# duckietown/gym-duckietown

Hardware: NVIDIA H100
Metric: env-steps/sec (obs+reward+done) at N envs, 1/2/4/8 H100 vs CPU ref (higher is better)
Workload: dtype f64 logic / f32 raster / u8 obs

## Files before the change

gym-duckietown_b200/csrc/dts_render.cu:

```cuda
#include <algorithm>
#include <cstddef>
#include <cstdlib>
#include <type_traits>
#include <vector>

#include "dts_camera.cuh"
#include "dts_kernels.h"

namespace dts {

struct FishTab {
  const int32_t* src_xy;
  const short4* cbox;
  const short4* fbox;
  const int32_t* cell_start;
  const uint16_t* cell_bins;
  const int32_t* home_start;
  const int4* home_ent;
  int ext_x, ext_y;
};

struct PilTab {
  int W, H, ow, oh;
  int tx, ty;
// ... 357 lines not shown
    cur ^= 1;
    __syncwarp();
    if (n < 3) return;
  }
  const Vtx* P = g.poly[cur];
  if (lane + 2 < n) setup_and_emit(ec, P[0], P[lane + 1], P[lane + 2], id, tex, lat);
  __syncwarp();
}

__device__ __forceinline__ void process_triangle_uniform(const EmitCtx& ec, const Vtx& a, const Vtx& b, const Vtx& c,
                                                         int id, int tex, int lat, int lane) {
  const int cls = classify(a, b, c);
  if (cls == 2) return;
  if (cls == 0) { if (lane == 0) setup_and_emit(ec, a, b, c, id, tex, lat); }
  else clip_and_emit_warp(ec, a, b, c, id, tex, lat, lane);
}

__device__ __forceinline__ void process_triangle_lanes(const EmitCtx& ec, bool have, const Vtx& a, const Vtx& b,
                                                       const Vtx& c, int id, int tex, int lat, int lane) {
  const int cls = have ? classify(a, b, c) : 2;
  if (cls == 0) setup_and_emit(ec, a, b, c, id, tex, lat);
  unsigned need = __ballot_sync(0xffffffffu, cls == 1);
  while (need) {
    const int src = __ffs(need) - 1;
    need &= need - 1;
    Vtx va, vb, vc;
    const float* fa = reinterpret_cast<const float*>(&a);
    const float* fb = reinterpret_cast<const float*>(&b);
    const float* fc = reinterpret_cast<const float*>(&c);
#pragma unroll
    for (int k = 0; k < 9; k++) {
      reinterpret_cast<float*>(&va)[k] = __shfl_sync(0xffffffffu, fa[k], src);
      reinterpret_cast<float*>(&vb)[k] = __shfl_sync(0xffffffffu, fb[k], src);
      reinterpret_cast<float*>(&vc)[k] = __shfl_sync(0xffffffffu, fc[k], src);
    }
    const int sid = __shfl_sync(0xffffffffu, id, src), stex = __shfl_sync(0xffffffffu, tex, src);
    clip_and_emit_warp(ec, va, vb, vc, sid, stex, lat, lane);
  }
}

__device__ __forceinline__ bool box_overlaps(const int qx[4], const int qy[4], int n, int x_lo, int x_hi, int y_lo, int y_hi) {
#pragma unroll
  for (int k = 0; k < 4; k++) {
    if (k >= n) break;
    const int k1 = (k + 1) & 3;
    const int dx = qx[k1] - qx[k], dy = qy[k1] - qy[k];
    const int xs = (-dy > 0) ? x_hi : x_lo;
    const int ys = (dx > 0) ? y_hi : y_lo;
    const long long e = (long long)dx * (ys - qy[k]) - (long long)dy * (xs - qx[k]);
    if (e < 0) return false;
  }
  return true;
}
__device__ __forceinline__ bool bin_overlaps(const int qx[4], const int qy[4], int n, int ox, int oy) {
  return box_overlaps(qx, qy, n, ox + 8, ox + (kCoarseW - 1) * kSub + 56, oy + 8, oy + (kCoarseH - 1) * kSub + 56);
}

constexpr unsigned kRecGround = 0x100u;
constexpr unsigned kRecFlatOk = 0x200u;
__device__ __forceinline__ unsigned build_binrec(const PrimRec* __restrict__ pr, int p, int ox, int oy, BinRec* __restrict__ out,
                                                 const short4* __restrict__ fb = nullptr) {
  const int4 w0 = __ldg(reinterpret_cast<const int4*>(pr));
  const int4 w1 = __ldg(reinterpret_cast<const int4*>(pr) + 1);
  const float4 w2 = __ldg(reinterpret_cast<const float4*>(pr) + 2);
  const int ltq = __ldg(&pr->ltq);
  const int quad = (ltq >> 24) & 1;
  const int flat = (ltq & 0xffff) ? kKindFlat : 0;
  const int qx[4] = {w0.x, w0.z, w1.x, w1.z}, qy[4] = {w0.y, w0.w, w1.y, w1.w};
  const int nv = quad ? 4 : 3;
  unsigned live = 0xffu, inside = 0xffu;
  int E0[4] = {0, 0, 0, 0}, A[4] = {0, 0, 0, 0}, B[4] = {0, 0, 0, 0};
#pragma unroll
  for (int k = 0; k < 4; k++) {
    if (k >= nv) break;
    const int ka = k, kb = (k + 1) & 3;
    const int dx = qx[kb] - qx[ka], dy = qy[kb] - qy[ka];
    const int bias = (dy > 0 || (dy == 0 && dx < 0)) ? 0 : 1;
    long long e0 = (long long)dx * (oy - qy[ka]) - (long long)dy * (ox - qx[ka]) - bias;
    if (e0 < -(1LL << 30)) live = 0;
    if (e0 > (1LL << 30)) e0 = (1LL << 30);
    if (e0 < -(1LL << 30)) e0 = -(1LL << 30);
    const int a = -dy, b = dx, e = (int)e0;
    E0[k] = e; A[k] = a; B[k] = b;
    if (fb) {
    } else {
      const int hi = (a > 0 ? a * 504 : a * 8) + (b > 0 ? b * 248 : b * 8);
      const int lo = (a > 0 ? a * 8 : a * 504) + (b > 0 ? b * 8 : b * 248);
#pragma unroll
      for (int f = 0; f < 8; f++) {
        const int ef = e + a * ((f & 3) * kBinW * kSub) + b * ((f >> 2) * kBinH * kSub);
        if (ef + hi < 0) live &= ~(1u << f);
        if (ef + lo < 0) inside &= ~(1u << f);
      }
    }
  }
  if (fb) {
#pragma unroll 1
    for (int f = 0; f < 8; f++) {
      const short4 q = fb[f];
      if (q.z < q.x) { live &= ~(1u << f); continue; }
      const int X0 = q.x * kSub - ox + 8, X1 = q.z * kSub - ox + 56, Y0 = q.y * kSub - oy + 8, Y1 = q.w * kSub - oy + 56;
#pragma unroll
      for (int k = 0; k < 4; k++) {
        if (k >= nv) break;
        const int a = A[k], b = B[k], e = E0[k];
        const int hi = (a > 0 ? a * X1 : a * X0) + (b > 0 ? b * Y1 : b * Y0);
        const int lo = (a > 0 ? a * X0 : a * X1) + (b > 0 ? b * Y0 : b * Y1);
        if (e + hi < 0) live &= ~(1u << f);
        if (e + lo < 0) inside &= ~(1u << f);
      }
    }
  }
  int tiny = 0;
  if (!fb && !quad && live) {
    const int minx = min(qx[0], min(qx[1], qx[2])) - ox, maxx = max(qx[0], max(qx[1], qx[2])) - ox;
    const int miny = min(qy[0], min(qy[1], qy[2])) - oy, maxy = max(qy[0], max(qy[1], qy[2])) - oy;
    const int x0 = max(minx >> 6, 0), x1 = min(maxx >> 6, kCoarseW - 1), y0 = max(miny >> 6, 0), y1 = min(maxy >> 6, kCoarseH - 1);
    if (x1 - x0 < 4 && y1 - y0 < 4 && x1 >= x0 && y1 >= y0) {
      tiny = kKindTiny;
      E0[3] = x0 | (y0 << 16); A[3] = x1 | (y1 << 16);
    }
  }
  const int id = __float_as_int(w2.w);
  int4* o = reinterpret_cast<int4*>(out);
  o[0] = make_int4(E0[0], E0[1], E0[2], E0[3]);
  o[1] = make_int4(A[0], A[1], A[2], A[3]);
  o[2] = make_int4(B[0], B[1], B[2], B[3]);
  o[3] = make_int4(__float_as_int(w2.x), __float_as_int(w2.y), __float_as_int(w2.z), id);
  o[4] = make_int4(qx[0] - ox, qy[0] - oy, (int)((unsigned)p | (live << 16) | ((inside & live) << 24)),
                   (quad ? kKindQuad : 0) | (id < 2 ? kKindGround : 0) | tiny | flat);
  return (inside & live) | (id < 2 ? kRecGround : 0u) | ((flat || id < 2) && !tiny ? kRecFlatOk : 0u);
}

struct ShadeIn {
  const PrimRec* pr;
  int x0, y0;
  float q0, qx, qy, u0, ux, uy, v0, vx, vy, r0;
  int ltq;
  unsigned tex;
};
__device__ __forceinline__ ShadeIn load_shade(const PrimRec* __restrict__ prims, unsigned w) {
  const PrimRec* pr = prims + w;
  const int2 xy0 = __ldg(reinterpret_cast<const int2*>(pr));
  const float4 w3 = __ldg(reinterpret_cast<const float4*>(pr) + 3);
  const float4 w4 = __ldg(reinterpret_cast<const float4*>(pr) + 4);
  const float4 w5 = __ldg(reinterpret_cast<const float4*>(pr) + 5);
  ShadeIn si;
  si.pr = pr; si.x0 = xy0.x; si.y0 = xy0.y;
  si.q0 = w3.x; si.qx = w3.y; si.qy = w3.z; si.u0 = w3.w;
  si.ux = w4.x; si.uy = w4.y; si.v0 = w4.z; si.vx = w4.w;
  si.vy = w5.x; si.ltq = __float_as_int(w5.y); si.tex = __float_as_uint(w5.z); si.r0 = w5.w;
  return si;
}
__device__ __forceinline__ void shade_eval(const ShadeIn& si, const uint8_t* __restrict__ tex_pool, const float4* __restrict__ lat_tab,
                                           int pxa, int pya, float c3[3]) {
  const float cdx = (float)(pxa + 32 - si.x0) * 0.015625f, cdy = (float)(pya + 32 - si.y0) * 0.015625f;
  float qq = fmaf(si.qy, cdy, fmaf(si.qx, cdx, si.q0));
  if (!(qq > 1e-20f)) qq = 1e-20f;
  const float rq = 1.0f / qq;
  const float u = fmaf(si.uy, cdy, fmaf(si.ux, cdx, si.u0)) * rq;
  const float v = fmaf(si.vy, cdy, fmaf(si.vx, cdx, si.v0)) * rq;
  const int ltq = si.ltq;
  const int lat = (ltq & 0xffff) - 1;
  if (lat >= 0) {
    const float fa_ = u * 7.0f, fb_ = (1.0f - v) * 7.0f;
    int ia = __float2int_rd(fa_), ib = __float2int_rd(fb_);
    ia = ia < 0 ? 0 : (ia > 6 ? 6 : ia);
    ib = ib < 0 ? 0 : (ib > 6 ? 6 : ib);
    const float fa = fa_ - (float)ia, fb = fb_ - (float)ib;
    const float4* L = lat_tab + lat * 64 + ia * 8 + ib;
    const bool lower = fb <= fa;
    const float4 c00 = L[0], c11 = L[9], cm = L[lower ? 8 : 1];
    const float t1 = lower ? fa : fb, t2 = lower ? fb : fa;
    c3[0] = fmaf(t2, c11.x - cm.x, fmaf(t1, cm.x - c00.x, c00.x));
    c3[1] = fmaf(t2, c11.y - cm.y, fmaf(t1, cm.y - c00.y, c00.y));
    c3[2] = fmaf(t2, c11.z - cm.z, fmaf(t1, cm.z - c00.z, c00.z));
  } else {
    const float4 w6 = __ldg(reinterpret_cast<const float4*>(si.pr) + 6);
    const float4 w7 = __ldg(reinterpret_cast<const float4*>(si.pr) + 7);
    c3[0] = fmaf(w6.y, cdy, fmaf(w6.x, cdx, si.r0)) * rq;
    c3[1] = fmaf(w7.x, cdy, fmaf(w6.w, cdx, w6.z)) * rq;
    c3[2] = fmaf(w7.w, cdy, fmaf(w7.z, cdx, w7.y)) * rq;
  }
  if (ltq & 0x00ff0000) {
    const unsigned ti = si.tex;
    const int lw = (ti >> 24) & 15, lh = ti >> 28;
    const int tw = 1 << lw, th = 1 << lh;
    const float twf = __int_as_float((127 + lw) << 23), thf = __int_as_float((127 + lh) << 23);
    const float tx = u * twf - 0.5f, ty = v * thf - 0.5f;
    const int txi = __float2int_rd(tx), tyi = __float2int_rd(ty);
    const float ffx = tx - (float)txi, ffy = ty - (float)tyi;
    const unsigned ti0 = (unsigned)txi & (tw - 1), ti1 = (ti0 + 1) & (tw - 1);
    const unsigned tj0 = (unsigned)tyi & (th - 1), tj1 = (tj0 + 1) & (th - 1);
    const unsigned r0 = tj0 << lw, r1 = tj1 << lw;
    const uchar4* tp = reinterpret_cast<const uchar4*>(tex_pool + ((size_t)(ti & 0xffffffu) << 8));
    const uchar4 t00 = __ldg(tp + (r0 + ti0)), t10 = __ldg(tp + (r0 + ti1));
    const uchar4 t01 = __ldg(tp + (r1 + ti0)), t11 = __ldg(tp + (r1 + ti1));
    const float a0[3] = {(float)t00.x, (float)t00.y, (float)t00.z}, a1[3] = {(float)t10.x, (float)t10.y, (float)t10.z};
    const float b0[3] = {(float)t01.x, (float)t01.y, (float)t01.z}, b1[3] = {(float)t11.x, (float)t11.y, (float)t11.z};
#pragma unroll
    for (int ch = 0; ch < 3; ch++) {
      const float ta = fmaf(ffx, a1[ch] - a0[ch], a0[ch]);
      const float tb = fmaf(ffx, b1[ch] - b0[ch], b0[ch]);
      const float tc = fmaf(ffy, tb - ta, ta);
      c3[ch] = tc * (c3[ch] * 0.00392156862745098f);
    }
  }
}
__device__ __forceinline__ void shade_prim(const PrimRec* __restrict__ prims, unsigned w, const uint8_t* __restrict__ tex_pool,
                                           const float4* __restrict__ lat_tab, int pxa, int pya, float c3[3]) {
  const ShadeIn si = load_shade(prims, w);
  shade_eval(si, tex_pool, lat_tab, pxa, pya, c3);
}

__device__ __forceinline__ uint32_t smem_u32(const void* p) { return (uint32_t)__cvta_generic_to_shared(p); }
__device__ __forceinline__ void mbar_init(uint64_t* bar, int count) {
  asm volatile("mbarrier.init.shared::cta.b64 [%0], %1;" ::"r"(smem_u32(bar)), "r"(count) : "memory");
}
__device__ __forceinline__ void mbar_fence_init() {
  asm volatile("fence.mbarrier_init.release.cluster;" ::: "memory");
  asm volatile("fence.proxy.async.shared::cta;" ::: "memory");
}
__device__ __forceinline__ void mbar_expect_tx(uint64_t* bar, uint32_t bytes) {
  asm volatile("mbarrier.arrive.expect_tx.shared::cta.b64 _, [%0], %1;" ::"r"(smem_u32(bar)), "r"(bytes) : "memory");
}
__device__ __forceinline__ void bulk_load(void* dst_smem, const void* src_gmem, uint32_t bytes, uint64_t* bar) {
  asm volatile("cp.async.bulk.shared::cluster.global.mbarrier::complete_tx::bytes [%0], [%1], %2, [%3];" ::"r"(smem_u32(dst_smem)),
               "l"(src_gmem), "r"(bytes), "r"(smem_u32(bar))
               : "memory");
}
__device__ __forceinline__ void mbar_wait(uint64_t* bar, uint32_t parity) {
  uint32_t ok;
  do {
    asm volatile("{\n .reg .pred p;\n mbarrier.try_wait.parity.shared::cta.b64 p, [%1], %2;\n selp.u32 %0, 1, 0, p;\n}"
                 : "=r"(ok)
                 : "r"(smem_u32(bar)), "r"(parity)
                 : "memory");
  } while (!ok);
}

__device__ __forceinline__ unsigned pack_rgb(float r, float g, float b) {
  const unsigned ur = min(__float2uint_rn(r * 255.0f), 255u);
  const unsigned ug = min(__float2uint_rn(g * 255.0f), 255u);
  const unsigned ub = min(__float2uint_rn(b * 255.0f), 255u);
  return ur | (ug << 8) | (ub << 16);
}

struct StoreLane {
  int src_lo, src_hi;
  int sh8;
  int off;
  int j, row;
};
__device__ __forceinline__ StoreLane make_store_lane(int lane, int W) {
  StoreLane sl;
  const int j = lane & 7, rowbase = lane & ~7;
  const int p0 = (4 * j) / 3;
  sl.sh8 = (4 * j - 3 * p0) * 8;
  sl.src_lo = rowbase + min(p0, 7);
  sl.src_hi = rowbase + min(p0 + 1, 7);
  sl.off = (lane >> 3) * W * 3 + 4 * j;
  sl.j = j; sl.row = lane >> 3;
  return sl;
}
__device__ __forceinline__ void store_bin_fast(uint8_t* __restrict__ bin0, const StoreLane& sl, unsigned rgb, int rows_ok) {
  const unsigned lo = __shfl_sync(0xffffffffu, rgb, sl.src_lo);
  const unsigned hi = __shfl_sync(0xffffffffu, rgb, sl.src_hi);
  const unsigned word = __funnelshift_r(lo | (hi << 24), hi >> 8, sl.sh8);
  if (sl.j < 6 && sl.row < rows_ok) *reinterpret_cast<unsigned*>(bin0 + sl.off) = word;
}
__device__ __forceinline__ void store_bin(uint8_t* __restrict__ out, unsigned rgb, int lane, int bx, int by, int W, int H) {
  const int gx = bx * kBinW + (lane & 7), gy = by * kBinH + (lane >> 3);
  if ((W & 3) == 0 && bx * kBinW + kBinW <= W) {
    const int j = lane & 7, rowbase = lane & ~7;
    const int p0 = (4 * j) / 3, sh8 = (4 * j - 3 * p0) * 8;
    const unsigned lo = __shfl_sync(0xffffffffu, rgb, rowbase + min(p0, 7));
    const unsigned hi = __shfl_sync(0xffffffffu, rgb, rowbase + min(p0 + 1, 7));
    const unsigned long long both = (unsigned long long)lo | ((unsigned long long)hi << 24);
    if (j < 6 && gy < H)
      *reinterpret_cast<unsigned*>(out + ((size_t)gy * W + bx * kBinW) * 3 + 4 * j) = (unsigned)(both >> sh8);
  } else if (gx < W && gy < H) {
    uint8_t* d = out + ((size_t)gy * W + gx) * 3;
    d[0] = (uint8_t)(rgb & 255); d[1] = (uint8_t)((rgb >> 8) & 255); d[2] = (uint8_t)(rgb >> 16);
  }
}

__device__ __forceinline__ size_t fmt_index(int layout, int x, int y, int c, int W, int H) {
  return layout == DTS_OBS_CHW ? ((size_t)c * H + y) * W + x
       : layout == DTS_OBS_CWH ? ((size_t)c * W + x) * H + y
                               : ((size_t)y * W + x) * 3 + c;
}
__device__ __forceinline__ void store_px_fmt(void* frame, int layout, int dtype, int x, int y, int W, int H, unsigned rgb) {
#pragma unroll
  for (int c = 0; c < 3; c++) {
    const unsigned v = (rgb >> (8 * c)) & 255u;
    const size_t i = fmt_index(layout, x, y, c, W, H);
    if (dtype == DTS_OBS_F32_UNIT) reinterpret_cast<float*>(frame)[i] = (float)v / 255.0f;
    else reinterpret_cast<uint8_t*>(frame)[i] = (uint8_t)v;
  }
}
__device__ __forceinline__ void store_bin_planar_u8(uint8_t* __restrict__ out, int layout, unsigned rgb, int lane, int bx, int by,
                                                    int W, int H) {
  const int j = lane < 24 ? lane : 0, c = j >> 3;
  int s0, step;
  size_t addr;
  if (layout == DTS_OBS_CHW) {
    const int r = (j & 7) >> 1, h = j & 1;
    s0 = r * 8 + 4 * h; step = 1;
    addr = ((size_t)c * H + by * kBinH + r) * W + bx * kBinW + 4 * h;
  } else {
    const int xi = j & 7;
    s0 = xi; step = 8;
    addr = ((size_t)c * W + bx * kBinW + xi) * H + by * kBinH;
  }
  const unsigned p0 = __shfl_sync(0xffffffffu, rgb, s0), p1 = __shfl_sync(0xffffffffu, rgb, s0 + step);
  const unsigned p2 = __shfl_sync(0xffffffffu, rgb, s0 + 2 * step), p3 = __shfl_sync(0xffffffffu, rgb, s0 + 3 * step);
  const unsigned sel = (unsigned)c | ((unsigned)(4 + c) << 4);
  const unsigned word = __byte_perm(__byte_perm(p0, p1, sel), __byte_perm(p2, p3, sel), 0x5410);
  if (lane < 24) *reinterpret_cast<unsigned*>(out + addr) = word;
}

__device__ __forceinline__ void store_bin_any(uint8_t* __restrict__ out, int fmt, unsigned rgb, int lane, int bx, int by,
                                              int W, int H) {
  if (fmt == 0) { store_bin(out, rgb, lane, bx, by, W, H); return; }
  const int gx = bx * kBinW + (lane & 7), gy = by * kBinH + (lane >> 3);
  if (gx < W && gy < H) store_px_fmt(out, fmt & 3, fmt >> 2, gx, gy, W, H, rgb);
}

__host__ __device__ __forceinline__ bool lean_output(int layout, int dtype, int W) {
  return layout == DTS_OBS_HWC && dtype == DTS_OBS_U8 && (W & 3) == 0;
}

__device__ __forceinline__ unsigned fine_rows_in_image(int cby, int H) { return ((cby * kCFY + 1) * kBinH < H) ? 0xffu : 0x0fu; }
__device__ __forceinline__ unsigned fine_in_image(int cbx, unsigned rows, int W) {
  const int nx = min(kCFX, (W - cbx * kCoarseW + kBinW - 1) / kBinW);
  const unsigned cols = (1u << nx) - 1u;
  return rows & (cols | (cols << 4));
}

struct FishPx { bool valid; int x, y; };
__device__ __forceinline__ FishPx fish_source(const FishTab& ft, int bx, int by, int lane, int W, int H) {
  const int gx = min(bx * kBinW + (lane & 7), W - 1), gy = min(by * kBinH + (lane >> 3), H - 1);
  const int sxy = __ldg(ft.src_xy + gy * W + gx);
  const int sx = (int)(short)(sxy & 0xffff), sy = sxy >> 16;
  return FishPx{sx != -32768, sx * kSub, sy * kSub};
}

__device__ __forceinline__ void store_bin_lean(uint8_t* __restrict__ out, const StoreLane& sl, unsigned rgb, int lane, int bx, int by,
                                               int W, int H) {
  if (bx * kBinW + kBinW <= W) store_bin_fast(out + ((size_t)(by * kBinH) * W + bx * kBinW) * 3, sl, rgb, min(kBinH, H - by * kBinH));
  else store_bin(out, rgb, lane, bx, by, W, H);
}

__device__ __forceinline__ void clear_colour(const DState& S, const RenderCfg& rc, int env, float clr[3]) {
  const bool seg = (rc.mode & DTS_RENDER_SEGMENT) != 0;
  clr[0] = seg ? 1.0f : S.rep[env].horizon[0];
  clr[1] = seg ? 0.0f : S.rep[env].horizon[1];
  clr[2] = seg ? 1.0f : S.rep[env].horizon[2];
}

__device__ __forceinline__ int n_listed(const int32_t* list, const int32_t* count, int n_envs) { return list ? __ldg(count) : n_envs; }
__device__ __forceinline__ int listed_env(const int32_t* list, int slot) { return list ? __ldg(list + slot) : slot; }

}

struct FrameMem {
  FrameCtx* ctx;
  PrimRec* prims;
  uint32_t* pairs;
  BinRec* recs;
  int* bin_count;
  int* bin_start;
  float4* lat;
  uint2* geo_list;
  uint2* solo;
  uint2* flat;
  int* work;
  int32_t* status;
};
constexpr int kWorkRaster = 0;
constexpr int kWorkPairPool = 1;
constexpr int kWorkGeoList = 2;
constexpr int kWorkSoloList = 3;
constexpr int kWorkFlatList = 4;

__host__ __device__ inline size_t align256(size_t b) { return (b + 255) & ~size_t(255); }

struct Renderer {
  int n, W, H, flags;
  int sms;
  int cbins;
  int max_prims = 0, max_lat = 0, items_max = 0, pool = 0;
  void* frame = nullptr;
  FrameMem fm{};
  FishTab fish{};
  FishTab rect{};
  PilTab pil{};
};

__host__ size_t carve(const Renderer& r, uintptr_t base, FrameMem& f) {
  const size_t n = r.n;
  size_t o = 0;
  auto take = [&](auto*& p, size_t count) {
    p = reinterpret_cast<std::remove_reference_t<decltype(p)>>(base + o);
    o += align256(count * sizeof(*p));
  };
  take(f.work, 64);
  take(f.ctx, n);
  take(f.bin_count, n * r.cbins);
  take(f.bin_start, n * r.cbins);
  take(f.prims, n * r.max_prims);
  take(f.pairs, r.pool);
  take(f.recs, r.pool);
  take(f.lat, n * r.max_lat * 64);
  take(f.geo_list, n * r.items_max);
  take(f.solo, n * r.cbins);
  take(f.flat, n * r.cbins);
  return o + 256;
}

__global__ void __launch_bounds__(128) k_frame_setup(const DState S, const DMap* __restrict__ maps, RenderCfg rc, FrameMem fm) {
  const int slot = blockIdx.x * blockDim.x + threadIdx.x;
  if (slot >= n_listed(rc.env_list, rc.env_count, rc.n_envs)) return;
  const int env = listed_env(rc.env_list, slot);
  FrameCtx& c = fm.ctx[env];
  const RenderEp ep = S.rep[env];
  double V[12];
  if (rc.mode & DTS_RENDER_TOP_DOWN) {
    const DMap& m = maps[S.map_id[env]];
    top_down_view((double)m.grid_w, (double)m.grid_h, m.tile_size, (double)ep.cam_fov_y_deg, V);
  } else {
    camera_view(S.pos_x[env], S.pos_z[env], S.angle[env], ep, (rc.flags & DTS_FLAG_DOMAIN_RAND) != 0, V);
  }
#pragma unroll
  for (int k = 0; k < 12; k++) c.V[k] = V[k];
  const double f = 1.0 / tan((double)ep.cam_fov_y_deg * kDeg2Rad / 2.0), aspect = (double)rc.width / (double)rc.height;
  const double zn = 0.04, zf = 100.0;
  c.P00 = (float)(f / aspect); c.P11 = (float)f;
  c.P22 = (float)((zf + zn) / (zn - zf)); c.P23 = (float)(2.0 * zf * zn / (zn - zf));
  c.n_prims = 0; c.n_lat = 0; c.overflow = 0; c.pad = 0;
}

__device__ __forceinline__ bool sphere_outside(float P00, float P11, float cx_, float cy_, float cz_, float rad) {
  const float hx = rsqrtf(P00 * P00 + 1.0f), hy = rsqrtf(P11 * P11 + 1.0f);
  bool out = cz_ - rad > -0.04f;
  out |= (P00 * cx_ + cz_) * hx > rad * 1.01f;
  out |= (-P00 * cx_ + cz_) * hx > rad * 1.01f;
  out |= (P11 * cy_ + cz_) * hy > rad * 1.01f;
  out |= (-P11 * cy_ + cz_) * hy > rad * 1.01f;
  return out;
}
__device__ __forceinline__ void eye_point(const double* V, double wx, double wy, double wz, float& ex, float& ey, float& ez) {
  ex = (float)(V[0] * wx + V[1] * wy + V[2] * wz + V[3]);
  ey = (float)(V[4] * wx + V[5] * wy + V[6] * wz + V[7]);
  ez = (float)(V[8] * wx + V[9] * wy + V[10] * wz + V[11]);
}

struct ItemPose { int dyn_kind; float opx, opz, orot; bool agent_item; };
__device__ __forceinline__ bool item_visible(const DState& S, const DMap& m, const RenderCfg& rc, const FrameCtx& ctx, int env,
                                             int item, ItemPose& ip) {
  const int n_tiles = m.grid_w * m.grid_h;
  ip.dyn_kind = 0; ip.opx = 0.f; ip.opz = 0.f; ip.orot = 0.f;
  ip.agent_item = item == agent_item(n_tiles, m.n_objects);
  if (item > agent_item(n_tiles, m.n_objects)) return false;
  if (ip.agent_item && (!(rc.mode & DTS_RENDER_TOP_DOWN) || m.agent.tri_count == 0)) return false;
  if (item >= 1 && item <= n_tiles) {
    const int t = item - 1, ti = t / m.grid_h, tj = t - ti * m.grid_h;
    if (m.tile_kind[tj * m.grid_w + ti] < 0) return false;
    const double ts = m.tile_size;
    float ex, ey, ez;
    eye_point(ctx.V, (ti + 0.5) * ts, 0.0, (tj + 0.5) * ts, ex, ey, ez);
    if (sphere_outside(ctx.P00, ctx.P11, ex, ey, ez, (float)(ts * 0.7071067811865476) * 1.001f + 1e-4f)) return false;
  } else if (item > n_tiles) {
    const int o = item - 1 - n_tiles;
    if (!ip.agent_item && (S.rep[env].hidden[o >> 5] >> (o & 31) & 1u)) return false;
    const DObject& ob = ip.agent_item ? m.agent : m.objects[o];
    ip.opx = ob.pos[0]; ip.opz = ob.pos[2]; ip.orot = ob.y_rot_deg;
    if (ip.agent_item) {
      ip.opx = (float)S.pos_x[env]; ip.opz = (float)S.pos_z[env];
      ip.orot = (float)(S.angle[env] * 180.0 / 3.141592653589793);
    }
    if (ob.dyn_slot >= 0) {
      ip.dyn_kind = m.dyn[ob.dyn_slot].kind;
      if (ip.dyn_kind != DTS_DYN_TRAFFICLIGHT) {
        const size_t nd = m.n_dyn, ne = rc.n_envs;
        ip.opx = (float)m.dyn_state[((size_t)DTS_DYN_PX * nd + ob.dyn_slot) * ne + env];
        ip.opz = (float)m.dyn_state[((size_t)DTS_DYN_PZ * nd + ob.dyn_slot) * ne + env];
        ip.orot = (float)m.dyn_state[((size_t)DTS_DYN_YROT * nd + ob.dyn_slot) * ne + env];
      }
    }
    double sn, cs;
    sincos((double)ip.orot * kDeg2Rad, &sn, &cs);
    const double sc = (double)ob.scale, ccx = ob.centre[0], ccy = ob.centre[1], ccz = ob.centre[2];
    float ex, ey, ez;
    eye_point(ctx.V, (double)ip.opx + sc * (cs * ccx + sn * ccz), (double)ob.pos[1] + sc * ccy, (double)ip.opz + sc * (-sn * ccx + cs * ccz), ex, ey, ez);
    if (sphere_outside(ctx.P00, ctx.P11, ex, ey, ez, ob.bound_rad * ob.scale * 1.002f + 2e-4f)) return false;
  }
  return true;
}

__global__ void __launch_bounds__(256) k_cull(const DState S, const DMap* __restrict__ maps, RenderCfg rc, FrameMem fm, int items_max,
                                              int32_t* __restrict__ err) {
  const size_t g = blockIdx.x * (size_t)blockDim.x + threadIdx.x;
  const int item = (int)(g / rc.n_envs), slot = (int)(g - (size_t)item * rc.n_envs);
  bool vis = false;
  int env = 0;
  if (item < items_max && slot < n_listed(rc.env_list, rc.env_count, rc.n_envs)) {
    env = listed_env(rc.env_list, slot);
    const DMap& m = maps[S.map_id[env]];
    ItemPose ip;
    vis = (rc.tessellate || item > m.grid_w * m.grid_h) && item_visible(S, m, rc, fm.ctx[env], env, item, ip);
  }
  const unsigned m = __ballot_sync(0xffffffffu, vis);
  if (!m) return;
  const int lane = threadIdx.x & 31;
  DTS_COUNT(28, __popc(m));
  int base = 0;
  if (lane == __ffs(m) - 1) base = atomicAdd(fm.work + kWorkGeoList, __popc(m));
  base = __shfl_sync(0xffffffffu, base, __ffs(m) - 1);
  if (vis) fm.geo_list[base + __popc(m & ((1u << lane) - 1u))] = make_uint2((unsigned)env, (unsigned)item);
}

__device__ __forceinline__ void load_geo_warp(GeoWarp& sh, const DState& S, const FrameCtx& ctx, int env, bool seg, int lane) {
  for (int k = lane; k < (int)(sizeof(RenderEp) / 4); k += 32)
    reinterpret_cast<uint32_t*>(&sh.ep)[k] = reinterpret_cast<const uint32_t*>(&S.rep[env])[k];
  if (lane < 12) sh.V[lane] = ctx.V[lane];
  if (lane == 12) { sh.P00 = ctx.P00; sh.P11 = ctx.P11; sh.P22 = ctx.P22; sh.P23 = ctx.P23; sh.unlit = seg ? 1 : 0; }
  __syncwarp();
}

__device__ __forceinline__ void draw_ground(const EmitCtx& ec, GeoWarp& sh, bool seg, int lane) {
  model_view(sh.V, 0.0, 0.0, 0.0, 1.0, 1.0, 0.0, sh.x, lane);
  const float gy = (float)(-0.8 * 0.01);
  const float P[4][3] = {{-50.f, gy, 50.f}, {-50.f, gy, -50.f}, {50.f, gy, -50.f}, {50.f, gy, 50.f}};
  const float magenta[3] = {255.f, 0.f, 255.f};
  const float* g = seg ? magenta : sh.ep.ground;
  const int pl_ = lane & 3;
// ... 659 lines not shown
            }
            bool coplanar = single && !(live_mask & ~ground_mask & ~flat_bits);
            if (coplanar && !simple) DTS_COUNT(20, 1);
            if (!simple) {
              if (first) {
#pragma unroll
                for (int s = 0; s < 4; s++) { z[s] = 1.0f; wn[s] = kNoPrim; }
                zb_used = false;
              }
#pragma unroll 1
              for (int phase = 0; phase < 2; phase++) {
                unsigned todo = phase == 0 ? (live_mask & ~ground_mask & ~tiny_bits) : ground_mask;
                if (phase == 1 && todo &&
                    __all_sync(0xffffffffu, wn[0] != kNoPrim && wn[1] != kNoPrim && wn[2] != kNoPrim && wn[3] != kNoPrim))
                  todo = 0;
                int seen = 0, twice = 0;
                while (todo) {
                  const int k = __ffs(todo) - 1;
                  todo &= todo - 1;
                  const BinRec& br = stage[k];
                  const uint32_t pflags = br.prim_flags;
                  DTS_COUNT(16, 1);
                  if ((pflags >> (24 + f)) & 1u) DTS_COUNT(17, 1);
                  int mask = 15;
                  if (!((pflags >> (24 + f)) & 1u)) {
                    mask = sample_mask(br, pxc, pyc);
                    if (!mask) continue;
                  }
                  if (coplanar && phase == 0) {
                    twice |= seen & mask;
                    seen |= mask;
#pragma unroll
                    for (int s = 0; s < 4; s++)
                      if (mask >> s & 1) wn[s] = pflags & 0xffffu;
                    continue;
                  }
                  const float4 zp = *reinterpret_cast<const float4*>(&br.z0);
                  const int2 xy0 = *reinterpret_cast<const int2*>(&br.x0);
                  const float cdx = (float)(pxc + 32 - xy0.x) * 0.015625f, cdy = (float)(pyc + 32 - xy0.y) * 0.015625f;
                  float zs[4];
                  int lt = 0, eq = 0;
#pragma unroll
                  for (int s = 0; s < 4; s++) {
                    const float sdx = cdx + (float)(sample_x(s) - 32) * 0.015625f, sdy = cdy + (float)(sample_y(s) - 32) * 0.015625f;
                    zs[s] = fmaf(zp.z, sdy, fmaf(zp.y, sdx, zp.x));
                    lt |= (zs[s] < z[s]) << s;
                    eq |= (zs[s] == z[s]) << s;
                  }
                  int pass_mask = mask & lt;
                  const int tie = mask & eq;
                  if (tie) {
                    const int my_id = __float_as_int(zp.w);
#pragma unroll
                    for (int s = 0; s < 4; s++)
                      if ((tie >> s & 1) && wn[s] != kNoPrim && my_id < __ldg(&prims[wn[s]].id)) pass_mask |= 1 << s;
                  }
                  if (!pass_mask) continue;
                  const unsigned me = pflags & 0xffffu;
#pragma unroll
                  for (int s = 0; s < 4; s++)
                    if (pass_mask >> s & 1) { z[s] = zs[s]; wn[s] = me; }
                }
                if (coplanar && phase == 0) {
                  if (__any_sync(0xffffffffu, twice != 0)) {
                    coplanar = false;
                    DTS_COUNT(21, 1);
#pragma unroll
                    for (int s = 0; s < 4; s++) wn[s] = kNoPrim;
                    phase = -1;
                  } else {
#pragma unroll
                    for (int s = 0; s < 4; s++)
                      if (seen >> s & 1) z[s] = -1.0f;
                  }
                }
              }
            }
            if (!kFish && !simple && (live_mask & tiny_bits)) {
              if (!zb_used) {
                zb_used = true;
#pragma unroll
                for (int s = 0; s < 4; s++) zb[lane * 4 + s] = ~0ull;
                __syncwarp();
              }
              DTS_COUNT(18, 1);
              DTS_COUNT(19, __popc(live_mask & tiny_bits));
              if ((live_mask & tiny_bits) >> lane & 1u) {
                const BinRec& br = stage[lane];
                const int4 E = *reinterpret_cast<const int4*>(br.E0);
                const int4 A = *reinterpret_cast<const int4*>(br.A);
                const int4 B = *reinterpret_cast<const int4*>(br.B);
                const float4 zp = *reinterpret_cast<const float4*>(&br.z0);
                const int2 xy0 = *reinterpret_cast<const int2*>(&br.x0);
                const int fx0 = (f & 3) * kBinW, fy0 = (f >> 2) * kBinH;
                const int x_lo = max(E.w & 0xffff, fx0), x_hi = min(A.w & 0xffff, fx0 + kBinW - 1);
                const int y_lo = max(E.w >> 16, fy0), y_hi = min(A.w >> 16, fy0 + kBinH - 1);
                const unsigned long long tail = ((unsigned long long)(unsigned)__float_as_int(zp.w) << 16) | (br.prim_flags & 0xffffu);
                for (int py = y_lo; py <= y_hi; py++)
                  for (int px = x_lo; px <= x_hi; px++) {
                    const int X = px * kSub, Y = py * kSub;
                    const int ec0 = E.x + A.x * X + B.x * Y, ec1 = E.y + A.y * X + B.y * Y, ec2 = E.z + A.z * X + B.z * Y;
#pragma unroll
                    for (int s = 0; s < 4; s++) {
                      const int e0 = ec0 + A.x * sample_x(s) + B.x * sample_y(s);
                      const int e1 = ec1 + A.y * sample_x(s) + B.y * sample_y(s);
                      const int e2 = ec2 + A.z * sample_x(s) + B.z * sample_y(s);
                      if ((e0 | e1 | e2) < 0) continue;
                      const float sdx = (float)(X + sample_x(s) - xy0.x) * 0.015625f, sdy = (float)(Y + sample_y(s) - xy0.y) * 0.015625f;
                      const float zs = fmaf(zp.z, sdy, fmaf(zp.y, sdx, zp.x));
                      atomicMin(&zb[((py - fy0) * kBinW + (px - fx0)) * 4 + s], ((unsigned long long)float_key(zs) << 32) | tail);
                    }
                  }
              }
              __syncwarp();
            }
            if (!(last || simple)) continue;
            if (!kFish && !simple && zb_used) {
#pragma unroll
              for (int s = 0; s < 4; s++) {
                const unsigned long long k = zb[lane * 4 + s];
                if (k == ~0ull) continue;
                const float zt = key_float((unsigned)(k >> 32));
                bool win = zt < z[s];
                if (zt == z[s] && wn[s] != kNoPrim) win = (int)((k >> 16) & 0xffffu) < __ldg(&prims[wn[s]].id);
                if (win) { z[s] = zt; wn[s] = (unsigned)(k & 0xffffu); }
              }
              __syncwarp();
            }
            DTS_COUNT(11, 1);
            unsigned rgb = shade_resolve(wn, simple, clr, prims, tex_pool, lat_tab, ox + pxc, oy + pyc, lane, err);
            if (kFish && !px_valid) rgb = 0u;
            emit(rgb, bx, by);
          }
        }
      }
    }
    if (gather_rows) {
      const int rows = min(kCoarseH, H - cby * kCoarseH);
      gather_rows_out(obs, gt, env_off + (size_t)cby * kCoarseH * W * 3, (size_t)rows * W * 3, lane);
    }
    work = __shfl_sync(0xffffffffu, next_work, 0);
  }
}

template <bool kFish>
__global__ void __launch_bounds__(kThreads, kSoloMinCtas) k_raster_solo(const DState S, const DMap* __restrict__ maps, RenderCfg rc, FrameMem fm,
                                                                        FishTab ft, uint8_t* __restrict__ obs, int max_prims, int max_lat) {
  const int W = rc.width, H = rc.height;
  const int cbins_x = (W + kCoarseW - 1) / kCoarseW;
  const int lane = threadIdx.x & 31;
  const StoreLane sl = make_store_lane(lane, W);
  const size_t frame_bytes = (size_t)W * H * 3;
  const int n = fm.work[kWorkSoloList];
  const int warps = (gridDim.x * blockDim.x) >> 5;
  for (int i = (blockIdx.x * blockDim.x + threadIdx.x) >> 5; i < n; i += warps) {
    const uint2 e = fm.solo[i];
    const int env = (int)e.x, b = (int)(e.y & 0xffffu);
    const unsigned p = e.y >> 16;
    const int cby = b / cbins_x, cbx = b - cby * cbins_x;
    const uint8_t* tex_pool = maps[S.map_id[env]].tex_pool;
    const float4* lat_tab = fm.lat + (size_t)env * max_lat * 64;
    const ShadeIn si = load_shade(fm.prims + (size_t)env * max_prims, p);
    uint8_t* out = obs + (size_t)env * frame_bytes;
    const int nx = min(kCFX, (W - cbx * kCoarseW + kBinW - 1) / kBinW);
    const int ny = ((cby * kCFY + 1) * kBinH < H) ? 2 : 1;
#pragma unroll 1
    for (int fy = 0; fy < ny; fy++)
#pragma unroll 1
    for (int fx = 0; fx < nx; fx++) {
      const int bx = cbx * kCFX + fx, by = cby * kCFY + fy;
      int pxa = (bx * kBinW + (lane & 7)) * kSub, pya = (by * kBinH + (lane >> 3)) * kSub;
      bool px_valid = true;
      if (kFish) {
        const FishPx src = fish_source(ft, bx, by, lane, W, H);
        px_valid = src.valid;
        pxa = src.x; pya = src.y;
      }
      float c3[3];
      shade_eval(si, tex_pool, lat_tab, pxa, pya, c3);
      unsigned rgb = pack_rgb(c3[0], c3[1], c3[2]);
      if (kFish && !px_valid) rgb = 0u;
      store_bin_lean(out, sl, rgb, lane, bx, by, W, H);
    }
  }
}

constexpr int kEdgeQ = 64;
template <bool kFish>
__global__ void __launch_bounds__(kThreads, kFlatMinCtas) k_raster_flat(const DState S, const DMap* __restrict__ maps, RenderCfg rc, FrameMem fm,
                                                                        FishTab ft, uint8_t* __restrict__ obs, int max_prims, int max_lat,
                                                                        int32_t* __restrict__ err) {
  __shared__ BinRec stages[kWarps][kStage];
  __shared__ unsigned bin_rgb[kWarps][kCFX * kCFY * 32];
  __shared__ uint4 edge_q[kWarps][2][kEdgeQ];
  const int W = rc.width, H = rc.height;
  const int cbins_x = (W + kCoarseW - 1) / kCoarseW, cbins = cbins_x * ((H + kCoarseH - 1) / kCoarseH);
  const int lane = threadIdx.x & 31;
  BinRec* stage = stages[threadIdx.x >> 5];
  unsigned* rgb_buf = bin_rgb[threadIdx.x >> 5];
  uint4 (*q)[kEdgeQ] = edge_q[threadIdx.x >> 5];
  const size_t frame_bytes = (size_t)W * H * 3;
  const int pxs = (lane & 7) * kSub, pys = (lane >> 3) * kSub;
  const int warps = (gridDim.x * blockDim.x) >> 5;
  for (int i = (blockIdx.x * blockDim.x + threadIdx.x) >> 5; i < __ldg(fm.work + kWorkFlatList); i += warps) {
    const uint2 e = fm.flat[i];
    const int env = (int)e.x, b = (int)(e.y & 0xffffu), count = (int)(e.y >> 16);
    const int cby = b / cbins_x, cbx = b - cby * cbins_x;
    DTS_COUNT(24, 1);
    uint2 mine = make_uint2(0u, 0u);
    __syncwarp();
    if (lane < count) {
      const int4* src = reinterpret_cast<const int4*>(fm.recs + fm.bin_start[(size_t)env * cbins + b] + lane);
      int4* dst = reinterpret_cast<int4*>(stage + lane);
      int4 v[5];
#pragma unroll
      for (int k = 0; k < 5; k++) v[k] = __ldg(src + k);
#pragma unroll
      for (int k = 0; k < 5; k++) dst[k] = v[k];
      mine = make_uint2((unsigned)v[4].z, (unsigned)v[4].w);
    }
    __syncwarp();
    const unsigned ground_bits = __ballot_sync(0xffffffffu, (mine.y & kKindGround) != 0u);
    const uint8_t* tex_pool = maps[S.map_id[env]].tex_pool;
    const PrimRec* prims = fm.prims + (size_t)env * max_prims;
    const float4* lat_tab = fm.lat + (size_t)env * max_lat * 64;
    uint8_t* out = obs + (size_t)env * frame_bytes;
    float clr[3];
    clear_colour(S, rc, env, clr);
    int ox = cbx * kCoarseW * kSub, oy = cby * kCoarseH * kSub;
    if (kFish) { const short4 cb = ft.cbox[b]; ox = cb.x * kSub; oy = cb.y * kSub; }
    const int nx = min(kCFX, (W - cbx * kCoarseW + kBinW - 1) / kBinW);
    const int ny = ((cby * kCFY + 1) * kBinH < H) ? 2 : 1;
    unsigned qs = 0;
    int f = 0;
#pragma unroll 1
    for (; f < kCFX * kCFY; f++) {
      if ((f & 3) >= nx || (f >> 2) >= ny) continue;
      const int bx = cbx * kCFX + (f & 3), by = cby * kCFY + (f >> 2);
      int pxc = pxs + (f & 3) * kBinW * kSub, pyc = pys + (f >> 2) * kBinH * kSub;
      bool px_valid = true;
      if (kFish) {
        const FishPx src = fish_source(ft, bx, by, lane, W, H);
        px_valid = src.valid;
        pxc = src.x - ox; pyc = src.y - oy;
      }
      const bool live = (mine.x >> (16 + f)) & 1u;
      const unsigned live_mask = __ballot_sync(0xffffffffu, live);
      const unsigned full_mask = __ballot_sync(0xffffffffu, live && ((mine.x >> (24 + f)) & 1u));
      const unsigned ground_mask = live_mask & ground_bits, tiles = live_mask & ~ground_mask;
      const unsigned pick = tiles ? tiles : live_mask;
      const bool simple = pick && !(pick & (pick - 1)) && (pick & full_mask);
      unsigned wn[4] = {kNoPrim, kNoPrim, kNoPrim, kNoPrim};
      if (simple) {
        const unsigned w = stage[__ffs(pick) - 1].prim_flags & 0xffffu;
        wn[0] = w; wn[1] = w; wn[2] = w; wn[3] = w;
      } else {
        int seen = 0, twice = 0;
        for (unsigned todo = tiles; todo; todo &= todo - 1) {
          const BinRec& br = stage[__ffs(todo) - 1];
          const uint32_t pflags = br.prim_flags;
          const int mask = ((pflags >> (24 + f)) & 1u) ? 15 : sample_mask(br, pxc, pyc);
          twice |= seen & mask;
          seen |= mask;
#pragma unroll
          for (int s = 0; s < 4; s++)
            if (mask >> s & 1) wn[s] = pflags & 0xffffu;
        }
        unsigned todo = __all_sync(0xffffffffu, seen == 15) ? 0u : ground_mask;
        for (; todo; todo &= todo - 1) {
          const BinRec& br = stage[__ffs(todo) - 1];
          const uint32_t pflags = br.prim_flags;
          const int mask = (((pflags >> (24 + f)) & 1u) ? 15 : sample_mask(br, pxc, pyc)) & ~(seen & 15);
          if (!mask) continue;
          twice |= (seen >> 4) & mask;
          seen |= mask << 4;
          const float4 zp = *reinterpret_cast<const float4*>(&br.z0);
          const int2 xy0 = *reinterpret_cast<const int2*>(&br.x0);
          const float cdx = (float)(pxc + 32 - xy0.x) * 0.015625f, cdy = (float)(pyc + 32 - xy0.y) * 0.015625f;
#pragma unroll
          for (int s = 0; s < 4; s++) {
            const float sdx = cdx + (float)(sample_x(s) - 32) * 0.015625f, sdy = cdy + (float)(sample_y(s) - 32) * 0.015625f;
            if ((mask >> s & 1) && fmaf(zp.z, sdy, fmaf(zp.y, sdx, zp.x)) < 1.0f) wn[s] = pflags & 0xffffu;
          }
        }
        if (__any_sync(0xffffffffu, twice != 0)) {
          DTS_COUNT(25, 1);
          if (lane == 0) fm.bin_count[(size_t)env * cbins + b] = count;
          break;
        }
      }
      float c3[3] = {clr[0], clr[1], clr[2]};
      if (wn[0] != kNoPrim) shade_prim(prims, wn[0], tex_pool, lat_tab, ox + pxc, oy + pyc, c3);
      const bool edge = px_valid && !(wn[1] == wn[0] && wn[2] == wn[0] && wn[3] == wn[0]);
      const unsigned edges = __ballot_sync(0xffffffffu, edge);
      const unsigned slot = f * 32 + lane;
      if (edge) {
        const int e = (qs + __popc(edges & ((1u << lane) - 1u))) & (kEdgeQ - 1);
        q[0][e] = make_uint4(slot, (unsigned)(ox + pxc), (unsigned)(oy + pyc), wn[0] | (wn[1] << 16));
        q[1][e] = make_uint4(wn[2] | (wn[3] << 16), __float_as_uint(c3[0]), __float_as_uint(c3[1]), __float_as_uint(c3[2]));
      } else {
        rgb_buf[slot] = (kFish && !px_valid) ? 0u : pack_rgb(c3[0], c3[1], c3[2]);
      }
      qs += __popc(edges);
      DTS_COUNT(26, __popc(edges));
#pragma unroll 1
      for (int nq = (qs & 0xffffu) - (qs >> 16); nq >= 32 || (nq > 0 && f == (ny - 1) * kCFX + nx - 1); nq = (qs & 0xffffu) - (qs >> 16)) {
        DTS_COUNT(27, 1);
        const int take = min(nq, 32);
        __syncwarp();
        unsigned qw[4] = {0u, 0u, 0u, 0u};
        float q3[3] = {0.f, 0.f, 0.f};
        unsigned qslot = 0u;
        int qx = 0, qy = 0;
        if (lane < take) {
          const int e = ((qs >> 16) + lane) & (kEdgeQ - 1);
          const uint4 a = q[0][e], c = q[1][e];
          qslot = a.x; qx = (int)a.y; qy = (int)a.z;
          qw[0] = a.w & 0xffffu; qw[1] = a.w >> 16; qw[2] = c.x & 0xffffu; qw[3] = c.x >> 16;
          q3[0] = __uint_as_float(c.y); q3[1] = __uint_as_float(c.z); q3[2] = __uint_as_float(c.w);
        }
        resolve_edge(qw, q3, clr, prims, tex_pool, lat_tab, qx, qy, lane, err);
        if (lane < take) rgb_buf[qslot] = pack_rgb(q3[0], q3[1], q3[2]);
        qs += (unsigned)take << 16;
        __syncwarp();
      }
    }
    if (f < kCFX * kCFY) continue;
    __syncwarp();
    const StoreLane sl = make_store_lane(lane, W);
#pragma unroll 1
    for (int f = 0; f < kCFX * kCFY; f++) {
      if ((f & 3) >= nx || (f >> 2) >= ny) continue;
      store_bin_lean(out, sl, rgb_buf[f * 32 + lane], lane, cbx * kCFX + (f & 3), cby * kCFY + (f >> 2), W, H);
    }
  }
}

__global__ void __launch_bounds__(256) k_resize(const uint8_t* __restrict__ src, int W, int H, int ow, int oh, int n_envs,
                                                const int16_t* __restrict__ xtab ,
                                                const int16_t* __restrict__ ytab , void* __restrict__ dst, int layout,
                                                int dtype, const int32_t* __restrict__ env_list, const int32_t* __restrict__ env_count) {
  const size_t total = (size_t)n_listed(env_list, env_count, n_envs) * ow * oh;
  for (size_t g = blockIdx.x * (size_t)blockDim.x + threadIdx.x; g < total; g += (size_t)gridDim.x * blockDim.x) {
    const int x = (int)(g % ow), y = (int)((g / ow) % oh);
    const size_t env = (size_t)listed_env(env_list, (int)(g / ((size_t)ow * oh)));
    const int4 xa = __ldg(reinterpret_cast<const int4*>(xtab + 8 * x)), ya = __ldg(reinterpret_cast<const int4*>(ytab + 8 * y));
    const int xi[4] = {(short)(xa.x & 0xffff), xa.x >> 16, (short)(xa.y & 0xffff), xa.y >> 16};
    const int xw[4] = {(short)(xa.z & 0xffff), xa.z >> 16, (short)(xa.w & 0xffff), xa.w >> 16};
    const int yi[4] = {(short)(ya.x & 0xffff), ya.x >> 16, (short)(ya.y & 0xffff), ya.y >> 16};
    const int yw[4] = {(short)(ya.z & 0xffff), ya.z >> 16, (short)(ya.w & 0xffff), ya.w >> 16};
    const uint8_t* frame = src + env * (size_t)W * H * 3;
    long long acc[3] = {0, 0, 0};
#pragma unroll
    for (int r = 0; r < 4; r++) {
      const uint8_t* row = frame + (size_t)yi[r] * W * 3;
      int h0 = 0, h1 = 0, h2 = 0;
#pragma unroll
// ... 633 lines not shown
```

Before: 2.658 million.

## Use atomic work stealing in solo/flat raster and shade two bin rows together

The solo and flat raster kernels stop striding over their work lists by a fixed warp index. Each warp now pulls its next item from new per-list atomic counters, prefetching the next index while it processes the current one, so uneven items balance across warps. shade_eval becomes a template over N pixels, and the solo kernel shades the two vertical bins of a coarse cell in one call to raise instruction-level parallelism. The cost is more registers, redundant shading when only one row is valid, and a dependence on the new counters being zeroed before each launch.

```diff
diff --git a/gym-duckietown_b200/csrc/dts_render.cu b/gym-duckietown_b200/csrc/dts_render.cu
--- a/gym-duckietown_b200/csrc/dts_render.cu
+++ b/gym-duckietown_b200/csrc/dts_render.cu
@@ -533,65 +533,82 @@
   si.vy = w5.x; si.ltq = __float_as_int(w5.y); si.tex = __float_as_uint(w5.z); si.r0 = w5.w;
   return si;
 }
+template <int N>
 __device__ __forceinline__ void shade_eval(const ShadeIn& si, const uint8_t* __restrict__ tex_pool, const float4* __restrict__ lat_tab,
-                                           int pxa, int pya, float c3[3]) {
-  const float cdx = (float)(pxa + 32 - si.x0) * 0.015625f, cdy = (float)(pya + 32 - si.y0) * 0.015625f;
-  float qq = fmaf(si.qy, cdy, fmaf(si.qx, cdx, si.q0));
-  if (!(qq > 1e-20f)) qq = 1e-20f;
-  const float rq = 1.0f / qq;
-  const float u = fmaf(si.uy, cdy, fmaf(si.ux, cdx, si.u0)) * rq;
-  const float v = fmaf(si.vy, cdy, fmaf(si.vx, cdx, si.v0)) * rq;
+                                           const int (&pxa)[N], const int (&pya)[N], float (&c3)[N][3]) {
+  float cdx[N], cdy[N], rq[N], u[N], v[N];
+#pragma unroll
+  for (int k = 0; k < N; k++) {
+    cdx[k] = (float)(pxa[k] + 32 - si.x0) * 0.015625f; cdy[k] = (float)(pya[k] + 32 - si.y0) * 0.015625f;
+    float qq = fmaf(si.qy, cdy[k], fmaf(si.qx, cdx[k], si.q0));
+    if (!(qq > 1e-20f)) qq = 1e-20f;
+    rq[k] = 1.0f / qq;
+    u[k] = fmaf(si.uy, cdy[k], fmaf(si.ux, cdx[k], si.u0)) * rq[k];
+    v[k] = fmaf(si.vy, cdy[k], fmaf(si.vx, cdx[k], si.v0)) * rq[k];
+  }
   const int ltq = si.ltq;
   const int lat = (ltq & 0xffff) - 1;
   if (lat >= 0) {
-    const float fa_ = u * 7.0f, fb_ = (1.0f - v) * 7.0f;
-    int ia = __float2int_rd(fa_), ib = __float2int_rd(fb_);
-    ia = ia < 0 ? 0 : (ia > 6 ? 6 : ia);
-    ib = ib < 0 ? 0 : (ib > 6 ? 6 : ib);
-    const float fa = fa_ - (float)ia, fb = fb_ - (float)ib;
-    const float4* L = lat_tab + lat * 64 + ia * 8 + ib;
-    const bool lower = fb <= fa;
-    const float4 c00 = L[0], c11 = L[9], cm = L[lower ? 8 : 1];
-    const float t1 = lower ? fa : fb, t2 = lower ? fb : fa;
-    c3[0] = fmaf(t2, c11.x - cm.x, fmaf(t1, cm.x - c00.x, c00.x));
-    c3[1] = fmaf(t2, c11.y - cm.y, fmaf(t1, cm.y - c00.y, c00.y));
-    c3[2] = fmaf(t2, c11.z - cm.z, fmaf(t1, cm.z - c00.z, c00.z));
+#pragma unroll
+    for (int k = 0; k < N; k++) {
+      const float fa_ = u[k] * 7.0f, fb_ = (1.0f - v[k]) * 7.0f;
+      int ia = __float2int_rd(fa_), ib = __float2int_rd(fb_);
+      ia = ia < 0 ? 0 : (ia > 6 ? 6 : ia);
+      ib = ib < 0 ? 0 : (ib > 6 ? 6 : ib);
+      const float fa = fa_ - (float)ia, fb = fb_ - (float)ib;
+      const float4* L = lat_tab + lat * 64 + ia * 8 + ib;
+      const bool lower = fb <= fa;
+      const float4 c00 = L[0], c11 = L[9], cm = L[lower ? 8 : 1];
+      const float t1 = lower ? fa : fb, t2 = lower ? fb : fa;
+      c3[k][0] = fmaf(t2, c11.x - cm.x, fmaf(t1, cm.x - c00.x, c00.x));
+      c3[k][1] = fmaf(t2, c11.y - cm.y, fmaf(t1, cm.y - c00.y, c00.y));
+      c3[k][2] = fmaf(t2, c11.z - cm.z, fmaf(t1, cm.z - c00.z, c00.z));
+    }
   } else {
     const float4 w6 = __ldg(reinterpret_cast<const float4*>(si.pr) + 6);
     const float4 w7 = __ldg(reinterpret_cast<const float4*>(si.pr) + 7);
-    c3[0] = fmaf(w6.y, cdy, fmaf(w6.x, cdx, si.r0)) * rq;
-    c3[1] = fmaf(w7.x, cdy, fmaf(w6.w, cdx, w6.z)) * rq;
-    c3[2] = fmaf(w7.w, cdy, fmaf(w7.z, cdx, w7.y)) * rq;
+#pragma unroll
+    for (int k = 0; k < N; k++) {
+      c3[k][0] = fmaf(w6.y, cdy[k], fmaf(w6.x, cdx[k], si.r0)) * rq[k];
+      c3[k][1] = fmaf(w7.x, cdy[k], fmaf(w6.w, cdx[k], w6.z)) * rq[k];
+      c3[k][2] = fmaf(w7.w, cdy[k], fmaf(w7.z, cdx[k], w7.y)) * rq[k];
+    }
   }
   if (ltq & 0x00ff0000) {
     const unsigned ti = si.tex;
     const int lw = (ti >> 24) & 15, lh = ti >> 28;
     const int tw = 1 << lw, th = 1 << lh;
     const float twf = __int_as_float((127 + lw) << 23), thf = __int_as_float((127 + lh) << 23);
-    const float tx = u * twf - 0.5f, ty = v * thf - 0.5f;
-    const int txi = __float2int_rd(tx), tyi = __float2int_rd(ty);
-    const float ffx = tx - (float)txi, ffy = ty - (float)tyi;
-    const unsigned ti0 = (unsigned)txi & (tw - 1), ti1 = (ti0 + 1) & (tw - 1);
-    const unsigned tj0 = (unsigned)tyi & (th - 1), tj1 = (tj0 + 1) & (th - 1);
-    const unsigned r0 = tj0 << lw, r1 = tj1 << lw;
     const uchar4* tp = reinterpret_cast<const uchar4*>(tex_pool + ((size_t)(ti & 0xffffffu) << 8));
-    const uchar4 t00 = __ldg(tp + (r0 + ti0)), t10 = __ldg(tp + (r0 + ti1));
-    const uchar4 t01 = __ldg(tp + (r1 + ti0)), t11 = __ldg(tp + (r1 + ti1));
-    const float a0[3] = {(float)t00.x, (float)t00.y, (float)t00.z}, a1[3] = {(float)t10.x, (float)t10.y, (float)t10.z};
-    const float b0[3] = {(float)t01.x, (float)t01.y, (float)t01.z}, b1[3] = {(float)t11.x, (float)t11.y, (float)t11.z};
-#pragma unroll
-    for (int ch = 0; ch < 3; ch++) {
-      const float ta = fmaf(ffx, a1[ch] - a0[ch], a0[ch]);
-      const float tb = fmaf(ffx, b1[ch] - b0[ch], b0[ch]);
-      const float tc = fmaf(ffy, tb - ta, ta);
-      c3[ch] = tc * (c3[ch] * 0.00392156862745098f);
+#pragma unroll
+    for (int k = 0; k < N; k++) {
+      const float tx = u[k] * twf - 0.5f, ty = v[k] * thf - 0.5f;
+      const int txi = __float2int_rd(tx), tyi = __float2int_rd(ty);
+      const float ffx = tx - (float)txi, ffy = ty - (float)tyi;
+      const unsigned ti0 = (unsigned)txi & (tw - 1), ti1 = (ti0 + 1) & (tw - 1);
+      const unsigned tj0 = (unsigned)tyi & (th - 1), tj1 = (tj0 + 1) & (th - 1);
+      const unsigned r0 = tj0 << lw, r1 = tj1 << lw;
+      const uchar4 t00 = __ldg(tp + (r0 + ti0)), t10 = __ldg(tp + (r0 + ti1));
+      const uchar4 t01 = __ldg(tp + (r1 + ti0)), t11 = __ldg(tp + (r1 + ti1));
+      const float a0[3] = {(float)t00.x, (float)t00.y, (float)t00.z}, a1[3] = {(float)t10.x, (float)t10.y, (float)t10.z};
+      const float b0[3] = {(float)t01.x, (float)t01.y, (float)t01.z}, b1[3] = {(float)t11.x, (float)t11.y, (float)t11.z};
+#pragma unroll
+      for (int ch = 0; ch < 3; ch++) {
+        const float ta = fmaf(ffx, a1[ch] - a0[ch], a0[ch]);
+        const float tb = fmaf(ffx, b1[ch] - b0[ch], b0[ch]);
+        const float tc = fmaf(ffy, tb - ta, ta);
+        c3[k][ch] = tc * (c3[k][ch] * 0.00392156862745098f);
+      }
     }
   }
 }
 __device__ __forceinline__ void shade_prim(const PrimRec* __restrict__ prims, unsigned w, const uint8_t* __restrict__ tex_pool,
                                            const float4* __restrict__ lat_tab, int pxa, int pya, float c3[3]) {
   const ShadeIn si = load_shade(prims, w);
-  shade_eval(si, tex_pool, lat_tab, pxa, pya, c3);
+  const int px[1] = {pxa}, py[1] = {pya};
+  float c[1][3];
+  shade_eval<1>(si, tex_pool, lat_tab, px, py, c);
+  c3[0] = c[0][0]; c3[1] = c[0][1]; c3[2] = c[0][2];
 }
 
 __device__ __forceinline__ uint32_t smem_u32(const void* p) { return (uint32_t)__cvta_generic_to_shared(p); }
@@ -764,6 +781,14 @@
 constexpr int kWorkGeoList = 2;
 constexpr int kWorkSoloList = 3;
 constexpr int kWorkFlatList = 4;
+constexpr int kWorkSoloNext = 5;
+constexpr int kWorkFlatNext = 6;
+
+__device__ __forceinline__ int warp_take(int* ctr, int lane) {
+  int v = 0;
+  if (lane == 0) v = atomicAdd(ctr, 1);
+  return __shfl_sync(0xffffffffu, v, 0);
+}
 
 __host__ __device__ inline size_t align256(size_t b) { return (b + 255) & ~size_t(255); }
 
@@ -1729,8 +1754,9 @@
   const StoreLane sl = make_store_lane(lane, W);
   const size_t frame_bytes = (size_t)W * H * 3;
   const int n = fm.work[kWorkSoloList];
-  const int warps = (gridDim.x * blockDim.x) >> 5;
-  for (int i = (blockIdx.x * blockDim.x + threadIdx.x) >> 5; i < n; i += warps) {
+  int next = 0;
+  for (int i = warp_take(fm.work + kWorkSoloNext, lane); i < n; i = __shfl_sync(0xffffffffu, next, 0)) {
+    if (lane == 0) next = atomicAdd(fm.work + kWorkSoloNext, 1);
     const uint2 e = fm.solo[i];
     const int env = (int)e.x, b = (int)(e.y & 0xffffu);
     const unsigned p = e.y >> 16;
@@ -1742,22 +1768,28 @@
     const int nx = min(kCFX, (W - cbx * kCoarseW + kBinW - 1) / kBinW);
     const int ny = ((cby * kCFY + 1) * kBinH < H) ? 2 : 1;
 #pragma unroll 1
-    for (int fy = 0; fy < ny; fy++)
-#pragma unroll 1
     for (int fx = 0; fx < nx; fx++) {
-      const int bx = cbx * kCFX + fx, by = cby * kCFY + fy;
-      int pxa = (bx * kBinW + (lane & 7)) * kSub, pya = (by * kBinH + (lane >> 3)) * kSub;
-      bool px_valid = true;
-      if (kFish) {
-        const FishPx src = fish_source(ft, bx, by, lane, W, H);
-        px_valid = src.valid;
-        pxa = src.x; pya = src.y;
-      }
-      float c3[3];
-      shade_eval(si, tex_pool, lat_tab, pxa, pya, c3);
-      unsigned rgb = pack_rgb(c3[0], c3[1], c3[2]);
-      if (kFish && !px_valid) rgb = 0u;
-      store_bin_lean(out, sl, rgb, lane, bx, by, W, H);
+      const int bx = cbx * kCFX + fx, by[2] = {cby * kCFY, cby * kCFY + ny - 1};
+      int pxa[2], pya[2];
+      bool px_valid[2] = {true, true};
+#pragma unroll
+      for (int k = 0; k < 2; k++) {
+        pxa[k] = (bx * kBinW + (lane & 7)) * kSub; pya[k] = (by[k] * kBinH + (lane >> 3)) * kSub;
+        if (kFish) {
+          const FishPx src = fish_source(ft, bx, by[k], lane, W, H);
+          px_valid[k] = src.valid;
+          pxa[k] = src.x; pya[k] = src.y;
+        }
+      }
+      float c3[2][3];
+      shade_eval<2>(si, tex_pool, lat_tab, pxa, pya, c3);
+#pragma unroll
+      for (int k = 0; k < 2; k++) {
+        if (k == 1 && ny == 1) break;
+        unsigned rgb = pack_rgb(c3[k][0], c3[k][1], c3[k][2]);
+        if (kFish && !px_valid[k]) rgb = 0u;
+        store_bin_lean(out, sl, rgb, lane, bx, by[k], W, H);
+      }
     }
   }
 }
@@ -1778,8 +1810,9 @@
   uint4 (*q)[kEdgeQ] = edge_q[threadIdx.x >> 5];
   const size_t frame_bytes = (size_t)W * H * 3;
   const int pxs = (lane & 7) * kSub, pys = (lane >> 3) * kSub;
-  const int warps = (gridDim.x * blockDim.x) >> 5;
-  for (int i = (blockIdx.x * blockDim.x + threadIdx.x) >> 5; i < __ldg(fm.work + kWorkFlatList); i += warps) {
+  int next = 0;
+  for (int i = warp_take(fm.work + kWorkFlatNext, lane); i < __ldg(fm.work + kWorkFlatList); i = __shfl_sync(0xffffffffu, next, 0)) {
+    if (lane == 0) next = atomicAdd(fm.work + kWorkFlatNext, 1);
     const uint2 e = fm.flat[i];
     const int env = (int)e.x, b = (int)(e.y & 0xffffu), count = (int)(e.y >> 16);
     const int cby = b / cbins_x, cbx = b - cby * cbins_x;
```

Result: faster. 2.879 million, median of 6 (+8.3%).
